# soldasim/BOSS.jl

Hardware: AMD Instinct MI355X
Metric: gp_posterior_updates_per_sec (+ acq_evals_per_sec), N=4096 d=8 fp64 (higher is better)
Workload: dtype f64; 1 GPU; d=8 synthetic blackbox, GaussianProcess(Matern52) surrogate, N=4096 fp64 posterior update + ExpectedImprovement over 8192 candidates per GPU (BASELINE.json configs[1]+[2]); N=4096, d=8, M_per_gpu=8192, kernel=matern52, parallelism=single GPU: no exchange

## Files before the change

boss.jl_amd/api.py:

```python
from __future__ import annotations

import ctypes as C
import os
from typing import Optional, Sequence

import numpy as np

_HERE = os.path.dirname(os.path.abspath(__file__))
LIB_PATH = os.environ.get("BOSS_LIB_PATH") or os.path.join(_HERE, "libbosship.so")

BOSS_OK, BOSS_E_INVALID, BOSS_E_NO_DEVICE, BOSS_E_NOT_PD, BOSS_E_NEG_VAR, BOSS_E_NOT_FITTED, BOSS_E_ALLOC = range(7)
KERNELS = {"matern32": 0, "matern52": 1, "sqexp": 2}
FIT_NO_SYNC = 1

_c_dp = C.POINTER(C.c_double)
_c_ucp = C.POINTER(C.c_ubyte)

SIGNATURES = {
    "boss_version": (C.c_char_p, []),
    "boss_last_error": (C.c_char_p, []),
    "boss_device_count": (C.c_int, [C.POINTER(C.c_int)]),
    "boss_set_stream": (C.c_int, [C.c_int, C.c_void_p]),
    "boss_device_sync": (C.c_int, [C.c_int]),
    "boss_gp_create": (C.c_int, [C.c_int, C.c_int, C.c_int, C.c_int, _c_dp, _c_dp, _c_ucp, C.POINTER(C.c_void_p)]),
# ... 1191 lines not shown
    return ch.value, tm.value, fb.value


def _fallbacks(device: int = 0):
    lib = load_library()
    fn = lib.boss_debug_fallbacks
    fn.restype = C.c_int
    fn.argtypes = [C.c_int, C.POINTER(C.c_long), C.POINTER(C.c_int)]
    n, off = C.c_long(0), C.c_int(0)
    _check(fn(device, C.byref(n), C.byref(off)))
    return n.value, off.value


def _set_launches(device: int = 0):
    lib = load_library()
    fn = lib.boss_debug_set_launches
    fn.restype = C.c_int
    fn.argtypes = [C.c_int, C.POINTER(C.c_long), C.POINTER(C.c_long)]
    a, b = C.c_long(0), C.c_long(0)
    fn(device, C.byref(a), C.byref(b))
    return a.value, b.value


def _set_grad_launches(device: int = 0):
    lib = load_library()
    fn = lib.boss_debug_set_grad_launches
    fn.restype = C.c_int
    fn.argtypes = [C.c_int, C.POINTER(C.c_long)]
    a = C.c_long(0)
    fn(device, C.byref(a))
    return a.value
```

boss.jl_amd/csrc/acq_kernels.hpp:

```cpp
#pragma once
#include "grad_kernels.hpp"

namespace boss {

constexpr int EI_MAXP = 16;
struct EiPar {
    int P, mode;
    double best;
    double coefs[EI_MAXP], ymax[EI_MAXP];
};

__device__ __forceinline__ double ei_value(const double* __restrict__ mu, const double* __restrict__ var, int ldm, int j,
                                           const EiPar& par, const double* __restrict__ coefs_dev,
                                           const double* __restrict__ ymax_dev) {
    const int P = par.P, mode = par.mode;
    if (mode == 0) return 0.0;
    double muf = 0.0, vf = 0.0, fp = 1.0;
    bool poison = false;
    for (int p = 0; p < P; ++p) {
        const double cf = (P <= EI_MAXP) ? par.coefs[p] : coefs_dev[p];
        const double ym = (mode & 2) ? ((P <= EI_MAXP) ? par.ymax[p] : ymax_dev[p]) : INFINITY;
        double m = mu[(size_t)p * ldm + j], v = var[(size_t)p * ldm + j];
        if (v < 0.0) {
            if (v >= -MAX_NEG_VAR) v = 0.0;
// ... 31 lines not shown
__global__ void ei_accumulate_kernel(const double* __restrict__ mu, const double* __restrict__ var, int ldm, int M,
                                     EiPar par, const double* __restrict__ coefs_dev,
                                     const double* __restrict__ ymax_dev, double* __restrict__ acq_sum) {
    const int j = blockIdx.x * blockDim.x + threadIdx.x;
    if (j >= M) return;
    acq_sum[j] += ei_value(mu, var, ldm, j, par, coefs_dev, ymax_dev);
}

__global__ void ei_accumulate_set_kernel(const double* __restrict__ mu, const double* __restrict__ var, size_t sstride, int ldm, int M,
                                         int s0, int s1, EiPar par, const double* __restrict__ coefs_dev,
                                         const double* __restrict__ ymax_dev, double* __restrict__ acq_sum) {
    const int j = blockIdx.x * blockDim.x + threadIdx.x;
    if (j >= M) return;
    double a = acq_sum[j];
    for (int s = s0; s < s1; ++s) a += ei_value(mu + (size_t)s * sstride, var + (size_t)s * sstride, ldm, j, par, coefs_dev, ymax_dev);
    acq_sum[j] = a;
}

__device__ __forceinline__ bool better(double a, long ia, double b, long ib) {
    const bool an = a != a, bn = b != b;
    if (an != bn) return an;
    if (!an && a != b) return a > b;
    return ia < ib;
}

constexpr int ACQ_EPI_THREADS = 1024;
__global__ __launch_bounds__(ACQ_EPI_THREADS) void acq_epilogue_kernel(const double* __restrict__ mu,
                                                                       const double* __restrict__ var, int ldm, int M,
                                                                       EiPar par, const double* __restrict__ coefs_dev,
                                                                       const double* __restrict__ ymax_dev,
                                                                       double* __restrict__ acq_sum, int have_prev,
                                                                       double inv_s, const unsigned char* __restrict__ mask,
                                                                       double* __restrict__ res, unsigned long long res_seq,
                                                                       double* __restrict__ dpair = nullptr, long idx_off = 0) {
    __shared__ double sv[ACQ_EPI_THREADS];
    __shared__ long si[ACQ_EPI_THREADS];
    constexpr long NONE = 0x7fffffffffffffffL;
    double bv = -INFINITY;
    long bi = NONE;
    for (int j = threadIdx.x; j < M; j += ACQ_EPI_THREADS) {
        double a = ei_value(mu, var, ldm, j, par, coefs_dev, ymax_dev);
        if (have_prev) a += acq_sum[j];
        a *= inv_s;
        if (mask && !mask[j]) a = 0.0;
        acq_sum[j] = a;
        if (bi == NONE || better(a, j, bv, bi)) { bv = a; bi = j; }
    }
    sv[threadIdx.x] = bv;
    si[threadIdx.x] = bi;
    __syncthreads();
    for (int st = ACQ_EPI_THREADS / 2; st > 0; st >>= 1) {
        if (threadIdx.x < st) {
            const double ov = sv[threadIdx.x + st];
            const long oi = si[threadIdx.x + st];
            if (oi != NONE && (si[threadIdx.x] == NONE || better(ov, oi, sv[threadIdx.x], si[threadIdx.x]))) {
                sv[threadIdx.x] = ov;
                si[threadIdx.x] = oi;
            }
        }
        __syncthreads();
    }
    if (threadIdx.x == 0) {
        if (dpair) {
            dpair[0] = sv[0];
            dpair[1] = (double)(si[0] + idx_off);
        }
        res[0] = sv[0];
        reinterpret_cast<long*>(res)[1] = si[0];
// ... 139 lines not shown
```

boss.jl_amd/csrc/bosship.hip:

```cpp
#include "../../include/bosship.h"

#include <hip/hip_runtime.h>

#include <algorithm>
#include <cmath>
#include <cstdint>
#include <cstdio>
#include <cstdlib>
#include <atomic>
#include <chrono>
#include <cstring>
#include <functional>
#include <limits>
#include <map>
#include <mutex>
#include <string>
#include <thread>
#include <vector>

#include "gp_kernels.hpp"
#include "potrf.hpp"
#include "chain.hpp"
#include "small_calls.hpp"
#include "rider.hpp"
// ... 54 lines not shown
    int logical = -1;
    hipStream_t own_stream = nullptr;
    hipStream_t stream = nullptr;
    hipStream_t side_stream = nullptr;
    std::vector<hipEvent_t> ev_panel, ev_rest;
    hipEvent_t ev_fork = nullptr, ev_up = nullptr;
    unsigned long long* sig_panel = nullptr;
    unsigned long long* sig_panel_host = nullptr;
    unsigned long long sig_seq = 0;
    hipStream_t chain_stream = nullptr, strip_stream = nullptr;
    unsigned long long chain_seq = 0, crit_seq = 0, up_seq = 0;
    int n_cus = 256;
    bool chain_ok = false;
    bool test_drop_chain = false;
    unsigned long long acq_seq = 0;
    unsigned long long few_seq = 0;
    std::mutex slab_mtx;
    void* slab_cache = nullptr;
    size_t slab_cache_bytes = 0;
    void* hostblk_cache = nullptr;
    size_t hostblk_cache_bytes = 0;
    unsigned long long* few_done = nullptr;
    unsigned long long few_done_cnt = 0;
    long set_launches = 0, set_pre_launches = 0;
    long set_grad_launches = 0;
    bool lookahead = true;
    bool prof_on = false;
    std::map<std::string, std::vector<std::pair<hipEvent_t, hipEvent_t>>> prof;
    std::vector<hipEvent_t> ev_pool;
    Workspace vscratch, csc, pred, acq, batchA, batchX, batchMisc, craw, lgA, lgB, lgC, few, setdesc, setmom, gsetdesc;
    static constexpr int LLG_BANKS = 4;
    Workspace lgbank[LLG_BANKS - 1][3];
    hipStream_t llg_stream[LLG_BANKS - 1] = {nullptr, nullptr, nullptr};
    hipEvent_t llg_join[LLG_BANKS - 1] = {nullptr, nullptr, nullptr};
    void* pinned = nullptr;
    struct TrailTab {
        TrailWork* dev = nullptr;
        std::vector<TrailWork> host;
        std::vector<int> off;
    };
    TrailTab trail[65];
    std::mutex mtx;
};

static void chain_quiesce(Ctx* c) {
    if (c->chain_stream) (void)hipStreamSynchronize(c->chain_stream);
// ... 40 lines not shown
    std::lock_guard<std::mutex> lk(g_ctx_mtx);
    auto it = g_ctx.find(device);
    if (all_out) *all_out = it != g_ctx.end() ? it->second->set_launches : 0;
    if (pre_out) *pre_out = it != g_ctx.end() ? it->second->set_pre_launches : 0;
    return BOSS_OK;
}

extern "C" int boss_debug_set_grad_launches(int device, long* out) {
    std::lock_guard<std::mutex> lk(g_ctx_mtx);
    auto it = g_ctx.find(device);
    if (out) *out = it != g_ctx.end() ? it->second->set_grad_launches : 0;
    return BOSS_OK;
}

static void ctx_destroy(Ctx* c) {
    if (!c) return;
    if (c->own_stream) (void)hipStreamDestroy(c->own_stream);
    if (c->side_stream) (void)hipStreamDestroy(c->side_stream);
    if (c->chain_stream) (void)hipStreamDestroy(c->chain_stream);
    if (c->strip_stream) (void)hipStreamDestroy(c->strip_stream);
    if (c->ev_fork) (void)hipEventDestroy(c->ev_fork);
    if (c->sig_panel && !c->sig_panel_host) (void)hipFree(c->sig_panel);
    if (c->few_done) (void)hipFree(c->few_done);
    for (auto& t : c->trail)
        if (t.dev) (void)hipFree(t.dev);
    if (c->slab_cache) (void)hipFree(c->slab_cache);
    if (c->hostblk_cache) (void)hipHostFree(c->hostblk_cache);
    if (c->ev_up) (void)hipEventDestroy(c->ev_up);
    for (int i = 0; i < Ctx::LLG_BANKS - 1; ++i) {
        if (c->llg_stream[i]) (void)hipStreamDestroy(c->llg_stream[i]);
        if (c->llg_join[i]) (void)hipEventDestroy(c->llg_join[i]);
    }
    if (c->pinned) (void)hipHostFree(c->pinned);
    delete c;
}

static int ctx_init(Ctx* c) {
    {
        int least = 0, greatest = 0;
        (void)hipDeviceGetStreamPriorityRange(&least, &greatest);
        static const int cu_mask = getenv("BOSS_CU_MASK") ? atoi(getenv("BOSS_CU_MASK")) : 0;
        if (cu_mask) {
            hipDeviceProp_t prop;
            HIPCHK(hipGetDeviceProperties(&prop, c->device));
            const int ncu = prop.multiProcessorCount, words = (ncu + 31) / 32;
            auto make = [&](hipStream_t* st, int lo, int hi) {
// ... 106 lines not shown
    HIPCHK(hipFuncSetAttribute((const void*)winv_gemv_kernel<2>, hipFuncAttributeMaxDynamicSharedMemorySize, 150 * 1024));
    HIPCHK(hipFuncSetAttribute((const void*)winv_gemv_kernel<4>, hipFuncAttributeMaxDynamicSharedMemorySize, 150 * 1024));
    HIPCHK(hipFuncSetAttribute((const void*)winv_args_kernel<1>, hipFuncAttributeMaxDynamicSharedMemorySize, 150 * 1024));
    HIPCHK(hipFuncSetAttribute((const void*)winv_args_kernel<2>, hipFuncAttributeMaxDynamicSharedMemorySize, 150 * 1024));
    HIPCHK(hipFuncSetAttribute((const void*)winv_args_kernel<4>, hipFuncAttributeMaxDynamicSharedMemorySize, 150 * 1024));
    HIPCHK(hipFuncSetAttribute((const void*)winv_args_kernel<1, true>, hipFuncAttributeMaxDynamicSharedMemorySize, 150 * 1024));
    HIPCHK(hipFuncSetAttribute((const void*)few_back_finish_kernel<PredG32>, hipFuncAttributeMaxDynamicSharedMemorySize,
                               PredictLds<PredG32>::BYTES));
    HIPCHK(hipFuncSetAttribute((const void*)few_w_kernel<PredG32>, hipFuncAttributeMaxDynamicSharedMemorySize, PredictLds<PredG32>::BYTES));
    HIPCHK(hipFuncSetAttribute((const void*)few_finish_kernel<PredG32>, hipFuncAttributeMaxDynamicSharedMemorySize,
                               PredictLds<PredG32>::BYTES));
    HIPCHK(hipFuncSetAttribute((const void*)linvt_kernel<PredG32>, hipFuncAttributeMaxDynamicSharedMemorySize,
                               PredictLds<PredG32>::BYTES));
    HIPCHK(hipFuncSetAttribute((const void*)backsolve_kernel<PredG32>, hipFuncAttributeMaxDynamicSharedMemorySize,
                               PredictLds<PredG32>::BYTES));
    HIPCHK(hipFuncSetAttribute((const void*)backsolve_set_kernel<PredG32>, hipFuncAttributeMaxDynamicSharedMemorySize,
                               PredictLds<PredG32>::BYTES));
    HIPCHK(hipFuncSetAttribute((const void*)grad_accum_set_kernel, hipFuncAttributeMaxDynamicSharedMemorySize, 150 * 1024));
    HIPCHK(hipFuncSetAttribute((const void*)predict_kernel<PredG64>, hipFuncAttributeMaxDynamicSharedMemorySize,
                               PredictLds<PredG64>::BYTES));
    HIPCHK(hipFuncSetAttribute((const void*)predict_kernel<PredG32, true>, hipFuncAttributeMaxDynamicSharedMemorySize,
                               PredictLds<PredG32>::BYTES));
    HIPCHK(hipFuncSetAttribute((const void*)predict_kernel<PredG64, true>, hipFuncAttributeMaxDynamicSharedMemorySize,
                               PredictLds<PredG64>::BYTES));
    return BOSS_OK;
}

static int virtual_devices() {
    static const int v = getenv("BOSS_VIRTUAL_DEVICES") ? std::max(0, atoi(getenv("BOSS_VIRTUAL_DEVICES"))) : 0;
    return v;
}
static int visible_devices(int* nphys_out = nullptr) {
    int n = 0;
    if (hipGetDeviceCount(&n) != hipSuccess || n <= 0) return 0;
    if (nphys_out) *nphys_out = n;
    return virtual_devices() > 0 ? virtual_devices() : n;
}

static int get_ctx(int device, Ctx** out) {
    std::lock_guard<std::mutex> lk(g_ctx_mtx);
    auto it = g_ctx.find(device);
    if (it != g_ctx.end()) {
        *out = it->second;
        HIPCHK(hipSetDevice(it->second->device));
        return BOSS_OK;
    }
// ... 180 lines not shown
    Ctx* c;
    int rc = get_ctx(device, &c);
    if (rc) return rc;
    HIPCHK(hipStreamSynchronize(c->stream));
    return BOSS_OK;
}

static bool few_done_ensure(Ctx* c, hipStream_t s) {
    if (c->few_done) return true;
    if (hipMalloc((void**)&c->few_done, sizeof(unsigned long long)) != hipSuccess) {
        (void)hipGetLastError();
        c->few_done = nullptr;
        return false;
    }
    (void)hipMemsetAsync(c->few_done, 0, sizeof(unsigned long long), s);
    c->few_done_cnt = 0;
    return true;
}
static bool few_fused() {
    static const bool v = !(getenv("BOSS_FEW_FUSED") && atoi(getenv("BOSS_FEW_FUSED")) == 0);
    return v;
}

#include "host_factor.inc"
#include "host_append.inc"
#include "host_batch.inc"
#include "host_predict.inc"
#include "host_acq.inc"
#include "host_rider.inc"
#include "host_track.inc"
#include "host_multi.inc"

extern "C" int boss_bench_mfma_f64(int device, int iters, double* tflops_out) {
    Ctx* c;
    int rc = get_ctx(device, &c);
    if (rc) return rc;
    hipDeviceProp_t prop;
    HIPCHK(hipGetDeviceProperties(&prop, device));
    const int blocks = prop.multiProcessorCount;
    double* sink;
    HIPCHK(dev_malloc((void**)&sink, 8));
    hipEvent_t e0, e1;
    HIPCHK(hipEventCreate(&e0));
    HIPCHK(hipEventCreate(&e1));
    hipLaunchKernelGGL(mfma_f64_rate_kernel, dim3(blocks), dim3(256), 0, c->stream, iters / 8 + 1, sink);
    HIPCHK(hipEventRecord(e0, c->stream));
// ... 130 lines not shown
```

boss.jl_amd/csrc/host_acq.inc:

```

static int acq_ei_impl(int P, int S, boss_gp_t* const* gps, const boss_cand_t* cand, const double* mean_Xs,
                       const double* fit_coefs, const double* y_max, int has_best, double best,
                       const unsigned char* valid_mask, double* acq_out, long* argmax_out, double* max_out,
                       double* dpair, long idx_off, bool defer) {
    if (P < 1 || S < 1 || !gps || !cand || !fit_coefs) return fail(BOSS_E_INVALID, "bad arguments");
    Ctx* c = cand->ctx;
    HIPCHK(hipSetDevice(c->device));
    for (int i = 0; i < P * S; ++i) {
        if (!gps[i]) return fail(BOSS_E_INVALID, "NULL posterior handle");
        if (gps[i]->ctx != c) return fail(BOSS_E_INVALID, "all handles and candidates must live on one device");
        if (!gps[i]->fitted) return fail(BOSS_E_NOT_FITTED, "handle has no valid factorisation");
    }
    std::lock_guard<std::mutex> lk(c->mtx);
    hipStream_t s = c->stream;
    const int M = cand->M;
    const size_t nd = (size_t)3 * P * M + M + 2 * P;
    {
        int rc = ws_reserve(c->acq, sizeof(double) * nd + M);
        if (rc) return rc;
    }
    double* dev = (double*)c->acq.p;
    double* dmu = dev;
    double* dvar = dmu + (size_t)P * M;
    double* dacq = dvar + (size_t)P * M;
    double* dmean = dacq + M;
    double* dcoef = dmean + (size_t)P * M;
    double* dymax = dcoef + P;
    unsigned char* dmask = (unsigned char*)(dev + nd);
    double* hres = (double*)c->pinned + (defer ? MULTI_RES_OFF : 0);
    EiPar par;
    int rc = ei_params(c, s, P, fit_coefs, y_max, has_best, best, &par, dcoef, dymax);
    if (rc) return rc;
    if (valid_mask) (void)hipMemcpyAsync(dmask, valid_mask, M, hipMemcpyHostToDevice, s);
    if (S > 1) (void)hipMemsetAsync(dacq, 0, sizeof(double) * M, s);
    std::vector<double> hmean;
    static const bool set_off = getenv("BOSS_NO_SET_PREDICT") && atoi(getenv("BOSS_NO_SET_PREDICT"));
    if (S > 1 && par.mode != 0 && !set_off && predict_set_ok(P * S, gps, cand)) {
        const size_t pm = (size_t)P * M;
        rc = ws_reserve(c->setmom, sizeof(double) * pm * S * (mean_Xs ? 3 : 2));
        if (rc) return rc;
        double* mu_all = (double*)c->setmom.p;
        double* var_all = mu_all + pm * S;
        double* mean_all = mean_Xs ? var_all + pm * S : nullptr;
        if (mean_Xs) {
            hmean.resize(pm * S);
            for (int sm = 0; sm < S; ++sm)
                for (int j = 0; j < M; ++j)
                    for (int p = 0; p < P; ++p) hmean[pm * sm + (size_t)p * M + j] = mean_Xs[p + (size_t)P * (j + (size_t)M * sm)];
            (void)hipMemcpyAsync(mean_all, hmean.data(), sizeof(double) * pm * S, hipMemcpyHostToDevice, s);
            (void)hipStreamSynchronize(s);
        }
        rc = predict_set_enqueue(P * S, gps, cand, mean_all, mu_all, var_all, (size_t)M);
        if (rc) {
            (void)hipStreamSynchronize(s);
            return rc;
        }
        hipLaunchKernelGGL(ei_accumulate_set_kernel, dim3((M + 255) / 256), dim3(256), 0, s, (const double*)mu_all, (const double*)var_all, pm, M, M,
                           0, S - 1, par, dcoef, dymax, dacq);
        hipLaunchKernelGGL(acq_epilogue_kernel, dim3(1), dim3(ACQ_EPI_THREADS), 0, s, (const double*)(mu_all + pm * (S - 1)),
                           (const double*)(var_all + pm * (S - 1)), M, M, par, dcoef, dymax, dacq, 1, 1.0 / S, valid_mask ? dmask : nullptr, hres,
                           (acq_out || defer) ? 0ull : ++c->acq_seq, dpair, idx_off);
    } else
    for (int sm = 0; sm < S; ++sm) {
        if (par.mode != 0) {
            if (mean_Xs) {
                hmean.resize((size_t)P * M);
                for (int j = 0; j < M; ++j)
                    for (int p = 0; p < P; ++p) hmean[(size_t)p * M + j] = mean_Xs[p + (size_t)P * (j + (size_t)M * sm)];
                (void)hipMemcpyAsync(dmean, hmean.data(), sizeof(double) * P * M, hipMemcpyHostToDevice, s);
                (void)hipStreamSynchronize(s);
            }
            for (int p = 0; p < P; ++p) {
                rc = predict_enqueue(gps[p + (size_t)P * sm], cand, mean_Xs ? dmean + (size_t)p * M : nullptr,
                                     dmu + (size_t)p * M, dvar + (size_t)p * M);
                if (rc) {
                    (void)hipStreamSynchronize(s);
                    return rc;
                }
            }
        }
        ProfScope ps(c, sm + 1 < S ? "ei" : "argmax");
        if (sm + 1 < S)
            hipLaunchKernelGGL(ei_accumulate_kernel, dim3((M + 255) / 256), dim3(256), 0, s, dmu, dvar, M, M, par, dcoef, dymax,
                               dacq);
        else
            hipLaunchKernelGGL(acq_epilogue_kernel, dim3(1), dim3(ACQ_EPI_THREADS), 0, s, dmu, dvar, M, M, par, dcoef, dymax,
                               dacq, S > 1 ? 1 : 0, 1.0 / S, valid_mask ? dmask : nullptr, hres, (acq_out || defer) ? 0ull : ++c->acq_seq,
                               dpair, idx_off);
    }
    if (acq_out) (void)hipMemcpyAsync(acq_out, dacq, sizeof(double) * M, hipMemcpyDeviceToHost, s);
    if (defer) {
        hipError_t e0 = hipGetLastError();
        return e0 == hipSuccess ? BOSS_OK : fail(BOSS_E_NO_DEVICE, hipGetErrorString(e0));
    }
    bool got = false;
    if (!acq_out) {
        volatile unsigned long long* seq = reinterpret_cast<volatile unsigned long long*>(hres) + 2;
        for (unsigned long i = 1;; ++i) {
            if (*seq == c->acq_seq) {
                got = true;
                break;
            }
            if ((i & 0x3fff) == 0 && hipStreamQuery(s) != hipErrorNotReady) break;
        }
        std::atomic_thread_fence(std::memory_order_acquire);
    }
    hipError_t e = got ? hipSuccess : hipStreamSynchronize(s);
    hipError_t e2 = hipGetLastError();
    if (e != hipSuccess) return fail(BOSS_E_NO_DEVICE, hipGetErrorString(e));
    if (e2 != hipSuccess) return fail(BOSS_E_NO_DEVICE, hipGetErrorString(e2));
    if (argmax_out) std::memcpy(argmax_out, &hres[1], sizeof(long));
    if (max_out) *max_out = hres[0];
    return BOSS_OK;
}

extern "C" int boss_acq_ei(int P, int S, boss_gp_t* const* gps, const boss_cand_t* cand, const double* mean_Xs,
                           const double* fit_coefs, const double* y_max, int has_best, double best,
                           const unsigned char* valid_mask, double* acq_out, long* argmax_out, double* max_out) {
    return acq_ei_impl(P, S, gps, cand, mean_Xs, fit_coefs, y_max, has_best, best, valid_mask, acq_out, argmax_out, max_out, nullptr, 0, false);
}

extern "C" int boss_acq_ei_moments(int device, int P, int S, int M, const double* mu, const double* var,
                                   const double* fit_coefs, const double* y_max, int has_best, double best,
                                   const unsigned char* valid_mask, double* acq_out, long* argmax_out,
                                   double* max_out) {
    if (P < 1 || S < 1 || M < 1 || !mu || !var || !fit_coefs) return fail(BOSS_E_INVALID, "bad arguments");
    Ctx* c;
    int rc = get_ctx(device, &c);
    if (rc) return rc;
    HIPCHK(hipSetDevice(c->device));
    std::lock_guard<std::mutex> lk(c->mtx);
    hipStream_t s = c->stream;
    const size_t pm = (size_t)P * M;
// ... 208 lines not shown
```

boss.jl_amd/csrc/host_predict.inc:

```

extern "C" int boss_cand_create(int device, int d, int M, const double* Xs, boss_cand_t** out) {
    if (!out) return fail(BOSS_E_INVALID, "out is NULL");
    *out = nullptr;
    if (d < 1 || M < 1 || !Xs) return fail(BOSS_E_INVALID, "need d >= 1, M >= 1 and non-NULL Xs");
    Ctx* c;
    int rc = get_ctx(device, &c);
    if (rc) return rc;
    boss_cand* cd = new boss_cand();
    cd->ctx = c;
    cd->d = d;
    cd->M = M;
    cd->Mp = round_up(M, 64);
    if (dev_malloc((void**)&cd->Craw, sizeof(double) * d * cd->Mp) != hipSuccess) {
        delete cd;
        return fail(BOSS_E_ALLOC, "device allocation failed");
    }
    std::vector<double> buf;
    pack_points(buf, Xs, d, M, cd->Mp, nullptr);
    HIPCHK(hipMemcpy(cd->Craw, buf.data(), sizeof(double) * d * cd->Mp, hipMemcpyHostToDevice));
    *out = cd;
    return BOSS_OK;
}

static int drain(Ctx* c, int rc) {
// ... 116 lines not shown
    if (g->d <= GIBBS_KSTAR_MAX_D)
        hipLaunchKernelGGL(gibbs_kstar_cols_kernel, dim3(g->Np / 256, tiles), dim3(256),
                           sizeof(double) * (2 * g->d * 32 + 32 + 2 * 8 * 256), s, (const double*)g->Xraw, (const double*)g->lamX,
                           (const double*)g->ampX, g->d, g->N, g->Np, (const double*)cd->Craw, clam_dev, camp_dev, cd->Mp, out);
    else
        hipLaunchKernelGGL(gibbs_kstar_kernel<32>, dim3(g->Np / 256, tiles), dim3(256), sizeof(double) * (2 * g->d + 1) * 32, s,
                           (const double*)g->Xraw, (const double*)g->lamX, (const double*)g->ampX, g->d, g->N, g->Np,
                           (const double*)cd->Craw, clam_dev, camp_dev, cd->Mp, out);
}

static void small_dinv(boss_gp* g, hipStream_t s) {
    dinv_join(g);
    if (g->have_dinv || g->dinv0_gen == g->factor_gen) return;
    hipLaunchKernelGGL(potrf_dinv_kernel, dim3(8, 1, 1), dim3(64), 0, s, g->A, g->ld, (size_t)0, g->inv16, (size_t)0, g->Dinv, (size_t)0);
    g->dinv0_gen = g->factor_gen;
}
static bool small_predict_ok(const boss_gp* g, int M) {
    const long long cap = std::min<long long>(16384, 1024LL * SMALL_MAX_N * SMALL_MAX_N / ((long long)g->N * g->N));
    return small_fit_ok(g->ctx, g->N, g->d) && M <= cap && !g->aug && !g->gibbs;
}

static int predict_enqueue(boss_gp* g, const boss_cand* cd, const double* mean_s_dev, double* mu, double* var,
                           bool for_grad = false, const double* clam_dev = nullptr, const double* camp_dev = nullptr,
                           bool need_v = false) {
    Ctx* c = g->ctx;
    hipStream_t s = c->stream;
    if (!g->fitted) return fail(BOSS_E_NOT_FITTED, "handle has no valid factorisation");
    if (g->gibbs && !clam_dev)
        return fail(BOSS_E_INVALID, "nonstationary posteriors predict through boss_ngp_predict (λ(x*), α(x*) are needed)");
    if (cd->ctx != c) return fail(BOSS_E_INVALID, "candidates and posterior live on different devices");
    if (cd->d != g->d) return fail(BOSS_E_INVALID, "candidate dimension differs from the model's x_dim");
    if (!for_grad && !need_v && small_predict_ok(g, cd->M)) {
        small_dinv(g, s);
        const int grid = std::min(512, (cd->M + SPG_WAVES - 1) / SPG_WAVES);
        hipLaunchKernelGGL(small_predict_grad_kernel<false>, dim3(grid), dim3(SPG_THREADS), SPG_LDS_BYTES, s, (const double*)g->Dinv,
                           (const double*)g->A, g->ld, g->Np, g->N, g->d, g->kernel, g->amp2, (const double*)g->Xsc, g->ldx,
                           (const double*)cd->Craw, cd->Mp, cd->M, (const double*)g->invlam, (const unsigned char*)g->discrete_dev,
                           mean_s_dev, (const double*)nullptr, mu, var, (double*)nullptr, (double*)nullptr);
        HIPCHK(hipGetLastError());
        return BOSS_OK;
    }
    bool joined = false;
    auto join_dinv = [&]() {
        if (!joined) dinv_join(g);
        joined = true;
    };
    if (!g->have_dinv) {
        join_dinv();
        ProfScope ps(c, "dinv");
        dinv_launch(g, s);
        g->have_dinv = true;
    }
    g->dinv_used = true;
    const int Mp = cd->Mp;
    const int BN = slab_bn(cd->M, for_grad);
    const int tiles = (cd->M + BN - 1) / BN;
    int rc = ws_reserve(c->csc, sizeof(double) * (size_t)g->d * Mp);
    if (rc) return rc;
    rc = ws_reserve(c->vscratch, sizeof(double) * (size_t)tiles * BN * g->Np * (for_grad ? 2 : 1));
    if (rc) return rc;
    double* Csc = (double*)c->csc.p;
    if (!g->gibbs)
        hipLaunchKernelGGL(scale_cand_kernel, dim3((Mp + 255) / 256), dim3(256), 0, s, cd->Craw, Csc, g->invlam,
                           g->discrete_dev, g->d, Mp);
#ifdef BOSS_EXPERIMENTS
    static const int dbg = getenv("BOSS_DBG") ? atoi(getenv("BOSS_DBG")) : 0;
#else
    constexpr int dbg = 0;
#endif
    static const bool no_few = getenv("BOSS_NO_FEW") && atoi(getenv("BOSS_NO_FEW"));
    static const int few_max_tiles = getenv("BOSS_FEW_MAX_TILES") ? atoi(getenv("BOSS_FEW_MAX_TILES")) : 128;
    const int ftiles = (cd->M + 31) / 32;
    const size_t aug_lds = sizeof(double) * ((size_t)g->d * (64 + 256) + g->d);
    if (ftiles <= few_max_tiles && g->Np >= 4 * PRED_RB && g->d <= 64 && !no_few && (BN == 32 || for_grad)) {
        typedef PredG32 G;
        typedef GemmDirect<4, 1, 2, 2, 8> GU;
        ProfScope ps(c, "predict");
        const int nb = g->Np / PRED_RB;
        const int nwg = g->Np / WINV_ROWS;
        const size_t step_part = (size_t)ftiles * nb * FEW_STEP_PARTS * 64;
        rc = ws_reserve(c->few, sizeof(double) * ((size_t)ftiles * ((size_t)g->Np * 32 + 64) + (size_t)nwg * 8 + step_part));
        if (rc) return rc;
        double* R = (double*)c->few.p;
        double* ssmz = R + (size_t)ftiles * g->Np * 32;
        double* part = ssmz + 64 * (size_t)ftiles + (size_t)nwg * 8;
        double* V = (double*)c->vscratch.p;
        static const int winv_after = getenv("BOSS_WINV_AFTER") ? atoi(getenv("BOSS_WINV_AFTER")) : 2;
        const size_t winv_lds = sizeof(double) * (size_t)g->Np * (cd->M == 1 ? 1 : cd->M == 2 ? 2 : WINV_MAX_M);
        if (winv_after > 0 && !g->have_winv && ++g->few_calls >= winv_after) {
            const size_t bytes = sizeof(double) * (size_t)g->ld * g->Np;
            bool ok = (g->Winv != nullptr || dev_malloc((void**)&g->Winv, bytes) == hipSuccess) &&
                      (g->Linv != nullptr || dev_malloc((void**)&g->Linv, bytes) == hipSuccess);
            if (ok) {
                join_dinv();
                linv_enqueue(g, s, g->Winv, g->Linv);
                g->have_winv = true;
            } else {
// ... 92 lines not shown
    if (g->aug || g->gibbs) {
        ProfScope ps(c, "predict");
        double* V = (double*)c->vscratch.p;
        if (g->aug)
            hipLaunchKernelGGL(aug_kstar_kernel, dim3(g->Np / 256, tiles), dim3(256), aug_lds, s, (const double*)g->Xraw, g->ldx, g->d,
                               g->npts, g->N, g->Np, (const double*)cd->Craw, Mp, g->kernel, g->amp2, (const double*)g->invlam, V, BN);
        else if (BN == 32)
            gibbs_kstar32_launch(g, cd, clam_dev, camp_dev, tiles, V, s);
        else
            hipLaunchKernelGGL(gibbs_kstar_kernel<64>, dim3(g->Np / 256, tiles), dim3(256), sizeof(double) * (2 * g->d + 1) * 64, s,
                               (const double*)g->Xraw, (const double*)g->lamX, (const double*)g->ampX, g->d, g->N, g->Np,
                               (const double*)cd->Craw, clam_dev, camp_dev, Mp, V);
        if (BN == 32) {
            typedef PredG32 G;
            hipLaunchKernelGGL((predict_kernel<G, true>), dim3(tiles), dim3(G::NTHREADS), PredictLds<G>::BYTES, s, g->A, g->ld, g->Np,
                               g->N, g->Dinv2, g->Xsc, Csc, g->d, Mp, g->kernel, g->amp2, V, mean_s_dev, cd->M, mu, var, dbg);
        } else {
            typedef PredG64 G;
            hipLaunchKernelGGL((predict_kernel<G, true>), dim3(tiles), dim3(G::NTHREADS), PredictLds<G>::BYTES, s, g->A, g->ld, g->Np,
                               g->N, g->Dinv, g->Xsc, Csc, g->d, Mp, g->kernel, g->amp2, V, mean_s_dev, cd->M, mu, var, dbg);
        }
        if (g->gibbs) hipLaunchKernelGGL(gibbs_var_kernel, dim3((cd->M + 255) / 256), dim3(256), 0, s, var, camp_dev, cd->M);
        HIPCHK(hipGetLastError());
        return BOSS_OK;
    }
    {
        ProfScope ps(c, "predict");
        if (BN == 32) {
            typedef PredG32 G;
            hipLaunchKernelGGL(predict_kernel<G>, dim3(tiles), dim3(G::NTHREADS), PredictLds<G>::BYTES, s, g->A, g->ld, g->Np,
                               g->N, g->Dinv2, g->Xsc, Csc, g->d, Mp, g->kernel, g->amp2, (double*)c->vscratch.p, mean_s_dev, cd->M, mu, var, dbg);
        } else {
            typedef PredG64 G;
            hipLaunchKernelGGL(predict_kernel<G>, dim3(tiles), dim3(G::NTHREADS), PredictLds<G>::BYTES, s, g->A, g->ld, g->Np,
                               g->N, g->Dinv, g->Xsc, Csc, g->d, Mp, g->kernel, g->amp2, (double*)c->vscratch.p, mean_s_dev, cd->M, mu, var, dbg);
        }
    }
    HIPCHK(hipGetLastError());
    return BOSS_OK;
}

__global__ void scale_cand_set_kernel(const double* __restrict__ Craw, const PredSet* __restrict__ sets,
                                      const unsigned char* __restrict__ discrete, int d, int Mp) {
    const PredSet ps = sets[blockIdx.y];
    double* Csc = const_cast<double*>(ps.Csc);
    const int j = blockIdx.x * blockDim.x + threadIdx.x;
// ... 1020 lines not shown
```

boss.jl_amd/csrc/predict_kernels.hpp:

```cpp
#pragma once
#include "gram_kernels.hpp"

namespace boss {

constexpr int PRED_CS_MAX_D = 16;
template <class G>
struct PredictLds {
    static constexpr int LDR = G::BN + 16;
    static constexpr int PART = 2 * G::TN * 4;
    static constexpr int BYTES = (G::BM * LDR + 2 * G::WR * G::BN + G::NTHREADS * PART + PRED_CS_MAX_D * G::BN) * 8;
};

template <class G, bool PRE>
__device__ __forceinline__ void predict_body(const double* __restrict__ A, int ld, int Np, int N,
                                             const double* __restrict__ Dinv,
                                             const double* __restrict__ Xsc,
                                             const double* __restrict__ Csc, int d, int Mp, int kern,
                                             double amp2, double* __restrict__ V,
                                             const double* __restrict__ mean_s, int M,
                                             double* __restrict__ mu_out, double* __restrict__ var_out, int dbg_arg, int tile) {
#ifdef BOSS_EXPERIMENTS
    const int dbg = dbg_arg;
#else
    constexpr int dbg = 0;
#endif
    static_assert(G::WC == 1 && (G::BM == BLK || G::BM == 2 * BLK), "waves stacked along a 128- or 256-row block");
    constexpr int RB = G::BM;
    extern __shared__ double lds[];
    constexpr int BN = G::BN, TM = G::TM, TN = G::TN, LDR = PredictLds<G>::LDR;
    double* Rs = lds;
    double* red = Rs + RB * LDR;
    const int tid = threadIdx.x, lane = tid & 63;
    const int wave = __builtin_amdgcn_readfirstlane(tid >> 6);
    const int wr = wave, wc = 0;
    const int c0 = tile * BN;
    const int nblk = Np / RB;

    double* part = red + 2 * G::WR * G::BN;
#pragma unroll
    for (int u = 0; u < 2 * TN * 4; ++u) part[u * G::NTHREADS + tid] = 0.0;
    double* cs = part + (size_t)G::NTHREADS * PredictLds<G>::PART;
    const bool cs_ok = !PRE && d <= PRED_CS_MAX_D;
    if (cs_ok) {
        for (int idx = tid; idx < d * BN; idx += G::NTHREADS) cs[idx] = Csc[(size_t)(idx / BN) * Mp + c0 + (idx % BN)];
        __syncthreads();
    }

    for (int ib = 0; ib < nblk; ++ib) {
        v4d acc[TM][TN];
#pragma unroll
        for (int m = 0; m < TM; ++m)
#pragma unroll
            for (int n = 0; n < TN; ++n) acc[m][n] = v4d{0.0, 0.0, 0.0, 0.0};
        if (!(dbg & 4)) G::template run<1>(A + (size_t)ib * RB, ld, V, BN, ib * RB, acc);

        double r2[TM][TN][4];
#pragma unroll
        for (int m = 0; m < TM; ++m)
#pragma unroll
            for (int n = 0; n < TN; ++n)
#pragma unroll
                for (int i = 0; i < 4; ++i) r2[m][n][i] = 0.0;
        if (cs_ok && !(dbg & 1)) {
            for (int kd0 = 0; kd0 < d; kd0 += 4) {
                double xr[4][TM];
#pragma unroll
                for (int kk = 0; kk < 4; ++kk)
// ... 79 lines not shown
                    ps[0] = __builtin_fma(v, v, ps[0]);
                    ps[G::NTHREADS] = __builtin_fma(v, zr, ps[G::NTHREADS]);
                }
        }
        __syncthreads();
    }
#pragma unroll
    for (int n = 0; n < TN; ++n)
#pragma unroll
        for (int i = 0; i < 4; ++i) {
            double s = part[(size_t)(2 * (n * 4 + i)) * G::NTHREADS + tid], z = part[(size_t)(2 * (n * 4 + i) + 1) * G::NTHREADS + tid];
#pragma unroll
            for (int off = 1; off < 16; off <<= 1) {
                s += __shfl_xor(s, off);
                z += __shfl_xor(z, off);
            }
            if ((lane & 15) == 0) {
                const int col = G::col_of(wc, n, i, lane);
                red[wr * BN + col] = s;
                red[G::WR * BN + wr * BN + col] = z;
            }
        }
    __syncthreads();
    if (tid < BN) {
        double s = 0.0, z = 0.0;
#pragma unroll
        for (int w = 0; w < G::WR; ++w) {
            s += red[w * BN + tid];
            z += red[G::WR * BN + w * BN + tid];
        }
        const int j = c0 + tid;
        if (j < M) {
            mu_out[j] = (mean_s ? mean_s[j] : 0.0) + z;
            if constexpr (PRE) var_out[j] = (kern == KERN_GIBBS) ? -s
                                                                 : fmax(0.0, amp2 - s);
            else var_out[j] = amp2 - s + PREDICT_JITTER;
        }
    }
}

template <class G, bool PRE = false>
__global__ __launch_bounds__(G::NTHREADS) __attribute__((amdgpu_waves_per_eu(1, 1))) void predict_kernel(const double* __restrict__ A, int ld, int Np, int N,
                                                      const double* __restrict__ Dinv,
                                                      const double* __restrict__ Xsc,
                                                      const double* __restrict__ Csc, int d, int Mp, int kern,
                                                      double amp2, double* __restrict__ Vscratch,
                                                      const double* __restrict__ mean_s, int M,
                                                      double* __restrict__ mu_out, double* __restrict__ var_out, int dbg_arg) {
    predict_body<G, PRE>(A, ld, Np, N, Dinv, Xsc, Csc, d, Mp, kern, amp2, Vscratch + (size_t)blockIdx.x * Np * G::BN, mean_s, M, mu_out,
                         var_out, dbg_arg, (int)blockIdx.x);
}

struct PredSet {
    const double* A;
    const double* Dinv;
    const double* Xsc;
    const double* Csc;
    const double* mean_s;
    const double* invlam;
    double* mu;
    double* var;
    double amp2;
    const double* Xraw;
    const double* lamX;
    const double* ampX;
    const double* clam;
    const double* camp;
};
template <class G, bool PRE = false>
__global__ __launch_bounds__(G::NTHREADS) __attribute__((amdgpu_waves_per_eu(1, 1))) void predict_kernel_set(const PredSet* __restrict__ sets, int ld, int Np, int N,
                                                      int d, int Mp, int kern, double* __restrict__ Vscratch, int M) {
    const PredSet ps = sets[blockIdx.y];
    predict_body<G, PRE>(ps.A, ld, Np, N, ps.Dinv, ps.Xsc, ps.Csc, d, Mp, kern, ps.amp2,
// ... 815 lines not shown
```

boss.jl_amd/csrc/small_calls.hpp:

```cpp
#pragma once
#include "potrf.hpp"

namespace boss {

struct AppendTail {
    double y, mean;
    int N0;
    const double* hyp;
    double *scal, *dz, *vout;
    int* info;
};
template <int MC, bool APPEND = false>
__global__ __launch_bounds__(256) void winv_args_kernel(FewCand par, const double* __restrict__ Xsc, int N, int d, int kern, double amp2,
                                                        const double* __restrict__ U, int ldu, int Np,
                                                        const double* __restrict__ Afac, int ld, const double* __restrict__ kst,
                                                        double* __restrict__ part,
                                                        unsigned long long* __restrict__ done, unsigned long long done_after,
                                                        double* __restrict__ host_out, unsigned long long seq, AppendTail tail = AppendTail()) {
    extern __shared__ double ks[];
    const int tid = threadIdx.x, lane = tid & 63, wave = tid >> 6;
    const int kb = (gridDim.x - 1 - blockIdx.x) * WINV_ROWS;
    constexpr int KU = 8;
    const int cend = kb + WINV_ROWS;
    if (kst) {
// ... 101 lines not shown
            host_out[1] = tail.scal[1];
            reinterpret_cast<int*>(host_out + 2)[0] = inf;
            __threadfence_system();
            __hip_atomic_store(reinterpret_cast<unsigned long long*>(host_out + 3), seq, __ATOMIC_RELAXED, __HIP_MEMORY_SCOPE_SYSTEM);
            return;
        }
        long long bad = -1;
        for (int j = 0; j < M; ++j) {
            const double s = red[(2 * j) * 256], z = red[(2 * j + 1) * 256];
            double v = amp2 - s + PREDICT_JITTER;
            if (!(v >= 0.0)) {
                if (v >= -MAX_NEG_VAR) v = 0.0;
                else if (bad < 0) bad = j;
            }
            host_out[j] = par.mean[j] + z;
            host_out[4 + j] = v;
        }
        reinterpret_cast<long long*>(host_out)[8] = bad;
        __threadfence_system();
        __hip_atomic_store(reinterpret_cast<unsigned long long*>(host_out) + 9, seq, __ATOMIC_RELAXED, __HIP_MEMORY_SCOPE_SYSTEM);
    }
}

}
```

Measured before the change: 899.3 updates/s.

## Fuse candidate scaling and EI argmax epilogue into the predict kernel

For the single-model, single-sample acquisition path, the predict kernel now scales raw candidates itself and computes EI per candidate. A last-block-done atomic counter lets the final workgroup reduce per-tile best pairs into the argmax result. This removes the separate scale_cand and acq_epilogue launches and their round trips. In exchange it adds an atomic counter, a cross-workgroup pairs buffer, and a host fallback that reruns the unfused path if the result sequence is not delivered.

```diff
diff --git a/boss.jl_amd/api.py b/boss.jl_amd/api.py
--- a/boss.jl_amd/api.py
+++ b/boss.jl_amd/api.py
@@ -1237,6 +1237,16 @@
     return a.value, b.value
 
 
+def _acq_fused(set: int = -1, device: int = 0):
+    lib = load_library()
+    fn = lib.boss_debug_acq_fused
+    fn.restype = C.c_int
+    fn.argtypes = [C.c_int, C.c_int, C.POINTER(C.c_long)]
+    n = C.c_long(0)
+    fn(device, set, C.byref(n))
+    return n.value
+
+
 def _set_grad_launches(device: int = 0):
     lib = load_library()
     fn = lib.boss_debug_set_grad_launches
diff --git a/boss.jl_amd/csrc/acq_kernels.hpp b/boss.jl_amd/csrc/acq_kernels.hpp
--- a/boss.jl_amd/csrc/acq_kernels.hpp
+++ b/boss.jl_amd/csrc/acq_kernels.hpp
@@ -77,6 +77,18 @@
     if (an != bn) return an;
     if (!an && a != b) return a > b;
     return ia < ib;
+}
+
+__device__ __forceinline__ double acq_point(const double* __restrict__ mu, const double* __restrict__ var, int ldm, int jm, int j,
+                                            const EiPar& par, const double* __restrict__ coefs_dev, const double* __restrict__ ymax_dev,
+                                            double* __restrict__ acq_sum, int have_prev, double inv_s,
+                                            const unsigned char* __restrict__ mask) {
+    double a = ei_value(mu, var, ldm, jm, par, coefs_dev, ymax_dev);
+    if (have_prev) a += acq_sum[j];
+    a *= inv_s;
+    if (mask && !mask[j]) a = 0.0;
+    acq_sum[j] = a;
+    return a;
 }
 
 constexpr int ACQ_EPI_THREADS = 1024;
@@ -94,11 +106,7 @@
     double bv = -INFINITY;
     long bi = NONE;
     for (int j = threadIdx.x; j < M; j += ACQ_EPI_THREADS) {
-        double a = ei_value(mu, var, ldm, j, par, coefs_dev, ymax_dev);
-        if (have_prev) a += acq_sum[j];
-        a *= inv_s;
-        if (mask && !mask[j]) a = 0.0;
-        acq_sum[j] = a;
+        const double a = acq_point(mu, var, ldm, j, j, par, coefs_dev, ymax_dev, acq_sum, have_prev, inv_s, mask);
         if (bi == NONE || better(a, j, bv, bi)) { bv = a; bi = j; }
     }
     sv[threadIdx.x] = bv;
diff --git a/boss.jl_amd/csrc/bosship.hip b/boss.jl_amd/csrc/bosship.hip
--- a/boss.jl_amd/csrc/bosship.hip
+++ b/boss.jl_amd/csrc/bosship.hip
@@ -100,6 +100,10 @@
     size_t hostblk_cache_bytes = 0;
     unsigned long long* few_done = nullptr;
     unsigned long long few_done_cnt = 0;
+    unsigned long long* acq_done = nullptr;
+    unsigned long long acq_done_cnt = 0;
+    Workspace acq_pairs;
+    long acq_fused_launches = 0;
     long set_launches = 0, set_pre_launches = 0;
     long set_grad_launches = 0;
     bool lookahead = true;
@@ -186,6 +190,7 @@
     if (c->ev_fork) (void)hipEventDestroy(c->ev_fork);
     if (c->sig_panel && !c->sig_panel_host) (void)hipFree(c->sig_panel);
     if (c->few_done) (void)hipFree(c->few_done);
+    if (c->acq_done) (void)hipFree(c->acq_done);
     for (auto& t : c->trail)
         if (t.dev) (void)hipFree(t.dev);
     if (c->slab_cache) (void)hipFree(c->slab_cache);
@@ -338,6 +343,10 @@
     HIPCHK(hipFuncSetAttribute((const void*)predict_kernel<PredG32, true>, hipFuncAttributeMaxDynamicSharedMemorySize,
                                PredictLds<PredG32>::BYTES));
     HIPCHK(hipFuncSetAttribute((const void*)predict_kernel<PredG64, true>, hipFuncAttributeMaxDynamicSharedMemorySize,
+                               PredictLds<PredG64>::BYTES));
+    HIPCHK(hipFuncSetAttribute((const void*)predict_kernel<PredG32, false, AcqTail>, hipFuncAttributeMaxDynamicSharedMemorySize,
+                               PredictLds<PredG32>::BYTES));
+    HIPCHK(hipFuncSetAttribute((const void*)predict_kernel<PredG64, false, AcqTail>, hipFuncAttributeMaxDynamicSharedMemorySize,
                                PredictLds<PredG64>::BYTES));
     return BOSS_OK;
 }
@@ -564,6 +573,35 @@
     return v;
 }
 
+static std::atomic<int> g_acq_fused{-1};
+static bool acq_fused() {
+    int v = g_acq_fused.load(std::memory_order_relaxed);
+    if (v < 0) {
+        v = !(getenv("BOSS_ACQ_FUSED") && atoi(getenv("BOSS_ACQ_FUSED")) == 0) ? 1 : 0;
+        g_acq_fused.store(v, std::memory_order_relaxed);
+    }
+    return v != 0;
+}
+static bool acq_done_ensure(Ctx* c, hipStream_t s, int tiles) {
+    if (ws_reserve(c->acq_pairs, sizeof(double) * 2 * (size_t)tiles) != BOSS_OK) return false;
+    if (c->acq_done) return true;
+    if (hipMalloc((void**)&c->acq_done, sizeof(unsigned long long)) != hipSuccess) {
+        (void)hipGetLastError();
+        c->acq_done = nullptr;
+        return false;
+    }
+    (void)hipMemsetAsync(c->acq_done, 0, sizeof(unsigned long long), s);
+    c->acq_done_cnt = 0;
+    return true;
+}
+extern "C" int boss_debug_acq_fused(int device, int set, long* launches_out) {
+    if (set >= 0) g_acq_fused.store(set ? 1 : 0, std::memory_order_relaxed);
+    std::lock_guard<std::mutex> lk(g_ctx_mtx);
+    auto it = g_ctx.find(device);
+    if (launches_out) *launches_out = it != g_ctx.end() ? it->second->acq_fused_launches : 0;
+    return BOSS_OK;
+}
+
 #include "host_factor.inc"
 #include "host_append.inc"
 #include "host_batch.inc"
diff --git a/boss.jl_amd/csrc/host_acq.inc b/boss.jl_amd/csrc/host_acq.inc
--- a/boss.jl_amd/csrc/host_acq.inc
+++ b/boss.jl_amd/csrc/host_acq.inc
@@ -2,7 +2,7 @@
 static int acq_ei_impl(int P, int S, boss_gp_t* const* gps, const boss_cand_t* cand, const double* mean_Xs,
                        const double* fit_coefs, const double* y_max, int has_best, double best,
                        const unsigned char* valid_mask, double* acq_out, long* argmax_out, double* max_out,
-                       double* dpair, long idx_off, bool defer) {
+                       double* dpair, long idx_off, bool defer, bool may_fuse = true) {
     if (P < 1 || S < 1 || !gps || !cand || !fit_coefs) return fail(BOSS_E_INVALID, "bad arguments");
     Ctx* c = cand->ctx;
     HIPCHK(hipSetDevice(c->device));
@@ -11,7 +11,7 @@
         if (gps[i]->ctx != c) return fail(BOSS_E_INVALID, "all handles and candidates must live on one device");
         if (!gps[i]->fitted) return fail(BOSS_E_NOT_FITTED, "handle has no valid factorisation");
     }
-    std::lock_guard<std::mutex> lk(c->mtx);
+    std::unique_lock<std::mutex> lk(c->mtx);
     hipStream_t s = c->stream;
     const int M = cand->M;
     const size_t nd = (size_t)3 * P * M + M + 2 * P;
@@ -34,6 +34,7 @@
     if (valid_mask) (void)hipMemcpyAsync(dmask, valid_mask, M, hipMemcpyHostToDevice, s);
     if (S > 1) (void)hipMemsetAsync(dacq, 0, sizeof(double) * M, s);
     std::vector<double> hmean;
+    bool fused = false;
     static const bool set_off = getenv("BOSS_NO_SET_PREDICT") && atoi(getenv("BOSS_NO_SET_PREDICT"));
     if (S > 1 && par.mode != 0 && !set_off && predict_set_ok(P * S, gps, cand)) {
         const size_t pm = (size_t)P * M;
@@ -62,6 +63,18 @@
                            (acq_out || defer) ? 0ull : ++c->acq_seq, dpair, idx_off);
     } else
     for (int sm = 0; sm < S; ++sm) {
+        AcqTail tail;
+        const bool try_fuse = P == 1 && S == 1 && par.mode != 0 && may_fuse && acq_fused();
+        tail.done = nullptr;
+        if (try_fuse) {
+            tail.par = par;
+            tail.mask = valid_mask ? dmask : nullptr;
+            tail.acq = dacq;
+            tail.res = hres;
+            tail.res_seq = defer ? 0ull : c->acq_seq + 1;
+            tail.dpair = dpair;
+            tail.idx_off = idx_off;
+        }
         if (par.mode != 0) {
             if (mean_Xs) {
                 hmean.resize((size_t)P * M);
@@ -72,12 +85,17 @@
             }
             for (int p = 0; p < P; ++p) {
                 rc = predict_enqueue(gps[p + (size_t)P * sm], cand, mean_Xs ? dmean + (size_t)p * M : nullptr,
-                                     dmu + (size_t)p * M, dvar + (size_t)p * M);
+                                     dmu + (size_t)p * M, dvar + (size_t)p * M, false, nullptr, nullptr, false, try_fuse ? &tail : nullptr);
                 if (rc) {
                     (void)hipStreamSynchronize(s);
                     return rc;
                 }
             }
+        }
+        if (tail.done) {
+            fused = true;
+            if (!defer) ++c->acq_seq;
+            continue;
         }
         ProfScope ps(c, sm + 1 < S ? "ei" : "argmax");
         if (sm + 1 < S)
@@ -109,6 +127,14 @@
     hipError_t e2 = hipGetLastError();
     if (e != hipSuccess) return fail(BOSS_E_NO_DEVICE, hipGetErrorString(e));
     if (e2 != hipSuccess) return fail(BOSS_E_NO_DEVICE, hipGetErrorString(e2));
+    if (fused && !got && *(reinterpret_cast<volatile unsigned long long*>(hres) + 2) != c->acq_seq) {
+        std::fprintf(stderr, "[bosship] the one-launch acquisition call did not deliver its result; repeating it with the epilogue launch\n");
+        (void)hipMemsetAsync(c->acq_done, 0, sizeof(unsigned long long), s);
+        c->acq_done_cnt = 0;
+        lk.unlock();
+        return acq_ei_impl(P, S, gps, cand, mean_Xs, fit_coefs, y_max, has_best, best, valid_mask, acq_out, argmax_out, max_out, dpair,
+                           idx_off, defer, false);
+    }
     if (argmax_out) std::memcpy(argmax_out, &hres[1], sizeof(long));
     if (max_out) *max_out = hres[0];
     return BOSS_OK;
diff --git a/boss.jl_amd/csrc/host_predict.inc b/boss.jl_amd/csrc/host_predict.inc
--- a/boss.jl_amd/csrc/host_predict.inc
+++ b/boss.jl_amd/csrc/host_predict.inc
@@ -162,7 +162,7 @@
 
 static int predict_enqueue(boss_gp* g, const boss_cand* cd, const double* mean_s_dev, double* mu, double* var,
                            bool for_grad = false, const double* clam_dev = nullptr, const double* camp_dev = nullptr,
-                           bool need_v = false) {
+                           bool need_v = false, AcqTail* tail = nullptr) {
     Ctx* c = g->ctx;
     hipStream_t s = c->stream;
     if (!g->fitted) return fail(BOSS_E_NOT_FITTED, "handle has no valid factorisation");
@@ -200,7 +200,12 @@
     rc = ws_reserve(c->vscratch, sizeof(double) * (size_t)tiles * BN * g->Np * (for_grad ? 2 : 1));
     if (rc) return rc;
     double* Csc = (double*)c->csc.p;
-    if (!g->gibbs)
+    static const bool no_few = getenv("BOSS_NO_FEW") && atoi(getenv("BOSS_NO_FEW"));
+    static const int few_max_tiles = getenv("BOSS_FEW_MAX_TILES") ? atoi(getenv("BOSS_FEW_MAX_TILES")) : 128;
+    const int ftiles = (cd->M + 31) / 32;
+    const bool few = ftiles <= few_max_tiles && g->Np >= 4 * PRED_RB && g->d <= 64 && !no_few && (BN == 32 || for_grad);
+    const bool with_tail = tail && !few && !g->aug && !g->gibbs && g->d <= PRED_CS_MAX_D && acq_done_ensure(c, s, tiles);
+    if (!g->gibbs && !with_tail)
         hipLaunchKernelGGL(scale_cand_kernel, dim3((Mp + 255) / 256), dim3(256), 0, s, cd->Craw, Csc, g->invlam,
                            g->discrete_dev, g->d, Mp);
 #ifdef BOSS_EXPERIMENTS
@@ -208,11 +213,8 @@
 #else
     constexpr int dbg = 0;
 #endif
-    static const bool no_few = getenv("BOSS_NO_FEW") && atoi(getenv("BOSS_NO_FEW"));
-    static const int few_max_tiles = getenv("BOSS_FEW_MAX_TILES") ? atoi(getenv("BOSS_FEW_MAX_TILES")) : 128;
-    const int ftiles = (cd->M + 31) / 32;
     const size_t aug_lds = sizeof(double) * ((size_t)g->d * (64 + 256) + g->d);
-    if (ftiles <= few_max_tiles && g->Np >= 4 * PRED_RB && g->d <= 64 && !no_few && (BN == 32 || for_grad)) {
+    if (few) {
         typedef PredG32 G;
         typedef GemmDirect<4, 1, 2, 2, 8> GU;
         ProfScope ps(c, "predict");
@@ -351,6 +353,34 @@
         }
         if (g->gibbs) hipLaunchKernelGGL(gibbs_var_kernel, dim3((cd->M + 255) / 256), dim3(256), 0, s, var, camp_dev, cd->M);
         HIPCHK(hipGetLastError());
+        return BOSS_OK;
+    }
+    if (with_tail) {
+        ProfScope ps(c, "predict");
+        tail->Craw = cd->Craw;
+        tail->invlam = g->invlam;
+        tail->discrete = g->discrete_dev;
+        tail->pairs = (double*)c->acq_pairs.p;
+        tail->done = c->acq_done;
+        tail->done_after = c->acq_done_cnt + (unsigned long long)tiles;
+        if (BN == 32) {
+            typedef PredG32 G;
+            hipLaunchKernelGGL((predict_kernel<G, false, AcqTail>), dim3(tiles), dim3(G::NTHREADS), PredictLds<G>::BYTES, s, g->A, g->ld, g->Np,
+                               g->N, g->Dinv2, g->Xsc, (const double*)nullptr, g->d, Mp, g->kernel, g->amp2, (double*)c->vscratch.p, mean_s_dev,
+                               cd->M, mu, var, dbg, *tail);
+        } else {
+            typedef PredG64 G;
+            hipLaunchKernelGGL((predict_kernel<G, false, AcqTail>), dim3(tiles), dim3(G::NTHREADS), PredictLds<G>::BYTES, s, g->A, g->ld, g->Np,
+                               g->N, g->Dinv, g->Xsc, (const double*)nullptr, g->d, Mp, g->kernel, g->amp2, (double*)c->vscratch.p, mean_s_dev,
+                               cd->M, mu, var, dbg, *tail);
+        }
+        const hipError_t e = hipGetLastError();
+        if (e != hipSuccess) {
+            tail->done = nullptr;
+            return fail(BOSS_E_NO_DEVICE, hipGetErrorString(e));
+        }
+        c->acq_done_cnt = tail->done_after;
+        ++c->acq_fused_launches;
         return BOSS_OK;
     }
     {
diff --git a/boss.jl_amd/csrc/predict_kernels.hpp b/boss.jl_amd/csrc/predict_kernels.hpp
--- a/boss.jl_amd/csrc/predict_kernels.hpp
+++ b/boss.jl_amd/csrc/predict_kernels.hpp
@@ -11,14 +11,19 @@
     static constexpr int BYTES = (G::BM * LDR + 2 * G::WR * G::BN + G::NTHREADS * PART + PRED_CS_MAX_D * G::BN) * 8;
 };
 
-template <class G, bool PRE>
+struct NoTail {
+    static constexpr bool ON = false;
+};
+template <class G, bool PRE, class TAIL = NoTail>
 __device__ __forceinline__ void predict_body(const double* __restrict__ A, int ld, int Np, int N,
                                              const double* __restrict__ Dinv,
                                              const double* __restrict__ Xsc,
                                              const double* __restrict__ Csc, int d, int Mp, int kern,
                                              double amp2, double* __restrict__ V,
                                              const double* __restrict__ mean_s, int M,
-                                             double* __restrict__ mu_out, double* __restrict__ var_out, int dbg_arg, int tile) {
+                                             double* __restrict__ mu_out, double* __restrict__ var_out, int dbg_arg, int tile,
+                                             const TAIL& tail = TAIL()) {
+    static_assert(!(TAIL::ON && PRE), "the acquisition tail belongs to the plain model's kernel");
 #ifdef BOSS_EXPERIMENTS
     const int dbg = dbg_arg;
 #else
@@ -42,7 +47,10 @@
     double* cs = part + (size_t)G::NTHREADS * PredictLds<G>::PART;
     const bool cs_ok = !PRE && d <= PRED_CS_MAX_D;
     if (cs_ok) {
-        for (int idx = tid; idx < d * BN; idx += G::NTHREADS) cs[idx] = Csc[(size_t)(idx / BN) * Mp + c0 + (idx % BN)];
+        for (int idx = tid; idx < d * BN; idx += G::NTHREADS) {
+            if constexpr (TAIL::ON) cs[idx] = tail.scaled(idx / BN, Mp, c0 + (idx % BN));
+            else cs[idx] = Csc[(size_t)(idx / BN) * Mp + c0 + (idx % BN)];
+        }
         __syncthreads();
     }
 
@@ -168,6 +176,7 @@
             }
         }
     __syncthreads();
+    double mu_j = 0.0, var_j = 0.0;
     if (tid < BN) {
         double s = 0.0, z = 0.0;
 #pragma unroll
@@ -177,24 +186,28 @@
         }
         const int j = c0 + tid;
         if (j < M) {
-            mu_out[j] = (mean_s ? mean_s[j] : 0.0) + z;
-            if constexpr (PRE) var_out[j] = (kern == KERN_GIBBS) ? -s
-                                                                 : fmax(0.0, amp2 - s);
-            else var_out[j] = amp2 - s + PREDICT_JITTER;
-        }
-    }
-}
-
-template <class G, bool PRE = false>
+            mu_j = (mean_s ? mean_s[j] : 0.0) + z;
+            if constexpr (PRE) var_j = (kern == KERN_GIBBS) ? -s
+                                                            : fmax(0.0, amp2 - s);
+            else var_j = amp2 - s + PREDICT_JITTER;
+            mu_out[j] = mu_j;
+            var_out[j] = var_j;
+        }
+    }
+    if constexpr (TAIL::ON) tail.template finish<BN>(tile, M, mu_j, var_j, reinterpret_cast<int*>(Rs));
+}
+
+template <class G, bool PRE = false, class TAIL = NoTail>
 __global__ __launch_bounds__(G::NTHREADS) __attribute__((amdgpu_waves_per_eu(1, 1))) void predict_kernel(const double* __restrict__ A, int ld, int Np, int N,
                                                       const double* __restrict__ Dinv,
                                                       const double* __restrict__ Xsc,
                                                       const double* __restrict__ Csc, int d, int Mp, int kern,
                                                       double amp2, double* __restrict__ Vscratch,
                                                       const double* __restrict__ mean_s, int M,
-                                                      double* __restrict__ mu_out, double* __restrict__ var_out, int dbg_arg) {
-    predict_body<G, PRE>(A, ld, Np, N, Dinv, Xsc, Csc, d, Mp, kern, amp2, Vscratch + (size_t)blockIdx.x * Np * G::BN, mean_s, M, mu_out,
-                         var_out, dbg_arg, (int)blockIdx.x);
+                                                      double* __restrict__ mu_out, double* __restrict__ var_out, int dbg_arg,
+                                                      TAIL tail = TAIL()) {
+    predict_body<G, PRE, TAIL>(A, ld, Np, N, Dinv, Xsc, Csc, d, Mp, kern, amp2, Vscratch + (size_t)blockIdx.x * Np * G::BN, mean_s, M,
+                               mu_out, var_out, dbg_arg, (int)blockIdx.x, tail);
 }
 
 struct PredSet {
diff --git a/boss.jl_amd/csrc/small_calls.hpp b/boss.jl_amd/csrc/small_calls.hpp
--- a/boss.jl_amd/csrc/small_calls.hpp
+++ b/boss.jl_amd/csrc/small_calls.hpp
@@ -1,5 +1,6 @@
 #pragma once
 #include "potrf.hpp"
+#include "acq_kernels.hpp"
 
 namespace boss {
 
@@ -147,4 +148,87 @@
     }
 }
 
+struct AcqTail {
+    static constexpr bool ON = true;
+    const double* Craw;
+    const double* invlam;
+    const unsigned char* discrete;
+    EiPar par;
+    const unsigned char* mask;
+    double* acq;
+    double* pairs;
+    unsigned long long* done;
+    unsigned long long done_after;
+    double* res;
+    unsigned long long res_seq;
+    double* dpair;
+    long idx_off;
+
+    __device__ __forceinline__ double scaled(int k, int Mp, int j) const {
+        double v = Craw[(size_t)k * Mp + j];
+        if (discrete && discrete[k]) v = rint(v);
+        return v * invlam[k];
+    }
+    template <int BN>
+    __device__ __forceinline__ void finish(int tile, int M, double mu_j, double var_j, int* flag) const {
+        static_assert(BN <= 64, "one wave holds the tile's candidates");
+        constexpr long NONE = 0x7fffffffffffffffL;
+        const int tid = threadIdx.x;
+        if (tid < 64) {
+            const int j = tile * BN + tid;
+            double bv = -INFINITY;
+            long bi = NONE;
+            if (tid < BN && j < M) {
+                bv = acq_point(&mu_j, &var_j, 1, 0, j, par, nullptr, nullptr, acq, 0, 1.0, mask);
+                bi = j;
+            }
+            wave_best(bv, bi);
+            if (tid == 0) {
+                st_sc1(pairs + 2 * (size_t)tile, bv);
+                st_sc1(pairs + 2 * (size_t)tile + 1, __longlong_as_double((long long)bi));
+                drain_stores();
+                const unsigned long long before = __hip_atomic_fetch_add(as_global(done), 1ull, __ATOMIC_RELAXED, __HIP_MEMORY_SCOPE_AGENT);
+                *(volatile lds_int_t*)flag = (before + 1 == done_after) ? 1 : 0;
+            }
+        }
+        __syncthreads();
+        if (*(volatile lds_int_t*)flag == 0 || tid >= 64) return;
+        double bv = -INFINITY;
+        long bi = NONE;
+        for (int w = tid; w < (int)gridDim.x; w += 64) {
+            const double v = ld_sc1(pairs + 2 * (size_t)w);
+            const long i = (long)__double_as_longlong(ld_sc1(pairs + 2 * (size_t)w + 1));
+            if (i != NONE && (bi == NONE || better(v, i, bv, bi))) {
+                bv = v;
+                bi = i;
+            }
+        }
+        wave_best(bv, bi);
+        if (tid == 0) {
+            if (dpair) {
+                dpair[0] = bv;
+                dpair[1] = (double)(bi + idx_off);
+            }
+            res[0] = bv;
+            reinterpret_cast<long*>(res)[1] = bi;
+            if (res_seq) {
+                __threadfence_system();
+                __hip_atomic_store(reinterpret_cast<unsigned long long*>(res) + 2, res_seq, __ATOMIC_RELAXED, __HIP_MEMORY_SCOPE_SYSTEM);
+            }
+        }
+    }
+    static __device__ __forceinline__ void wave_best(double& bv, long& bi) {
+        constexpr long NONE = 0x7fffffffffffffffL;
+#pragma unroll
+        for (int off = 32; off >= 1; off >>= 1) {
+            const double ov = __shfl_xor(bv, off);
+            const long oi = ((long)__shfl_xor((int)(bi >> 32), off) << 32) | (unsigned)__shfl_xor((int)(bi & 0xffffffffL), off);
+            if (oi != NONE && (bi == NONE || better(ov, oi, bv, bi))) {
+                bv = ov;
+                bi = oi;
+            }
+        }
+    }
+};
+
 }
```

Result: slower. 886.3 updates/s (-1.4%).
